# lorenzsp/EMRI_FrequencyDomainWaveforms

Measured on AMD Instinct MI355X. Metric: FD waveforms/sec (2 yr, dt=10 s, ~3000 modes) at 1/2/4/8 GPUs; mode-sum HBM GB/s, higher is better.
Workload: dtype f64

## Files before the change

emri_frequencydomainwaveforms_amd/csrc/emrifd.hip:

```cpp

#include "emrifd_layout.h"

#define EFD_VERSION 100

static thread_local std::string g_err;

int efdhip::fail(int code, const std::string& msg) {
    g_err = msg;
    return code;
}

namespace {

constexpr int NWAVE = TILE / 64;
constexpr int XCD_GROUP = 1024 / TILE;
constexpr int SEGWIN = TILE;
constexpr int PIECES = (int)sizeof(Item) / 16;
constexpr int B_PIECE = (int)offsetof(Item, b) / 16;
constexpr int ROUNDS = 2;
constexpr int NC = (ROUNDS * TILE) / PIECES;


__device__ __forceinline__ bool seg_hits_tile(int2 lh, int32_t tlo, int32_t thi) {
    return lh.y > tlo && lh.x < thi;
}

struct HitRecords {
    int p0, count;
};
__device__ __forceinline__ HitRecords hit_records(
    int sg, int64_t tile, int32_t tlo, int32_t thi, const int32_t* __restrict__ segbase,
    const int32_t* __restrict__ stb0, const int32_t* __restrict__ stb1,
    const int4* __restrict__ seginfo, const int4* __restrict__ ranges) {
    const int32_t sbase = segbase[sg];
    if (sbase != SEG_NO_STB) {
        const int q0 = stb0[sbase + tile], q1 = stb1[sbase + tile];
        return {q0, max(q1 - q0, 0)};
    }
    const int4 info = seginfo[sg];
    const int base = info.x, n = info.y, dir = info.z, sb = info.w;
    int lo = 0, hi = n;
    while (lo < hi) {
        const int mid = (lo + hi) >> 1;
        const int4 rg = ranges[base + (dir > 0 ? mid : n - 1 - mid)];
        if ((sb ? rg.w : rg.y) > tlo) hi = mid; else lo = mid + 1;
    }
    const int p0 = lo;
    hi = n;
    while (lo < hi) {
// ... 232 lines not shown
    const uint64_t m = x >= 64 ? ~0ull : ((1ull << (x & 63)) - 1ull);
    return x <= 0 ? 0ull : m;
}
__device__ __forceinline__ uint64_t lane_range_mask(int32_t lo, int32_t hi) {
    return lanes_below(hi) & ~lanes_below(lo);
}
struct RecSign {
    int32_t fdcls;
    int32_t shift;
    double kth;
    bool safe;
};
__device__ __forceinline__ RecSign rec_sign(uint32_t bits) {
    const bool fdneg = bits & 1u;
    RecSign r;
    r.safe = (bits & 2u) != 0;
    r.fdcls = fdneg ? 0x018 : 0x180;
    r.shift = fdneg ? -192 : 192;
    r.kth = fdneg ? -KTH0 / VS : KTH0 / VS;
    return r;
}
__device__ __forceinline__ uint64_t class_mask(double x, int32_t cls) {
    uint64_t m;
    asm volatile("v_cmp_class_f64_e64 %0, %1, %2" : "=s"(m) : "v"(x), "s"(cls));
    return m;
}
__device__ __forceinline__ double ftz_select(bool ok, double v) {
    return __hiloint2double(ok ? __double2hiint(v) : 0, __double2loint(v));
}
constexpr int HDR_HB = TILE_LANES < 1024 ? 10 : 11;
constexpr uint32_t HDR_HM = (1u << HDR_HB) - 1u;
constexpr int HDR_S = 2 * HDR_HB, HDR_J = 2 * HDR_HB + 1, HDR_FD = 2 * HDR_HB + 4;
static_assert(FAST_J < 8, "header: jser in 3 bits");
static_assert(TILE_LANES < 2048 && HDR_FD + 2 <= 32, "header: one 32-bit word");
__device__ __forceinline__ uint32_t hdr_pack(uint32_t lo, uint32_t hi, int s, int32_t jser,
                                             int32_t fdneg) {
    return lo | (hi << HDR_HB) | ((uint32_t)s << HDR_S) | ((uint32_t)jser << HDR_J) |
           ((uint32_t)fdneg << HDR_FD);
}
__device__ __forceinline__ int32_t hdr_lo(uint32_t ha) { return (int32_t)(ha & HDR_HM); }
__device__ __forceinline__ int32_t hdr_hi(uint32_t ha) {
    return (int32_t)((ha >> HDR_HB) & HDR_HM);
}
__device__ __forceinline__ int hdr_s(uint32_t ha) { return (int)((ha >> HDR_S) & 1u); }
__device__ __forceinline__ uint32_t hdr_jser(uint32_t ha) { return (ha >> HDR_J) & 7u; }
__device__ __forceinline__ uint32_t hdr_fdneg(uint32_t ha) { return (ha >> HDR_FD) & 3u; }
__device__ __forceinline__ uint32_t hdr_safe(uint32_t ha) { return (ha >> (HDR_FD + 1)) & 1u; }
__device__ __forceinline__ bool hdr_test(uint32_t ha, uint32_t mask) {
    asm volatile("" : "+s"(ha));
    return (ha & mask) != 0;
}
__device__ __forceinline__ bool hdr_j3(uint32_t ha) {
    asm volatile("" : "+s"(ha));
    return hdr_jser(ha) >= 3u;
}
__device__ __forceinline__ bool hdr_j4(uint32_t ha) {
    asm volatile("" : "+s"(ha));
    return hdr_jser(ha) >= 4u;
}
__device__ __forceinline__ void spa_simple(const Item* __restrict__ it, double sfk, double stfk,
                                           const double2* __restrict__ sct, const RecSign& rs,
                                           double& wr, double& wi, double& w) {
    const double u = sfk - it->gx;
    const double tt = fma(fma(fma(it->ic[0], u, it->ic[1]), u, it->ic[2]), u, it->ic[3]);
    w = tt - it->tj;
    const double ph = fma(fma(fma(it->ph[0], w, it->ph[1]), w, it->ph[2]), w, it->ph[3]);
    const double fd = fma(fma(it->fd[0], w, it->fd[1]), w, it->fd[2]);
// ... 340 lines not shown
#pragma unroll
            for (int rd = 0; rd < KEYCAP / (4 * TILE); ++rd) {
                const int pc = rd * TILE + tid;
                if (4 * pc < pre)
                    glds16(reinterpret_cast<const uint4*>(tkeys + (size_t)tile * KEYCAP) + pc,
                           reinterpret_cast<uint4*>(keys) + rd * TILE + wave * 64);
            }
        }
#pragma unroll
        for (int rd = 0; rd < SCTAB / TILE; ++rd)
            glds16(reinterpret_cast<const uint4*>(sctab_g) + rd * TILE + tid,
                   reinterpret_cast<uint4*>(sctab) + rd * TILE + wave * 64);
        __builtin_amdgcn_s_waitcnt(0x0f70);
        __syncthreads();
    }

    const int32_t w_lo = (int32_t)(tile * TILE_LANES + wave * 64 * BPL);
    const int32_t e_lo = w_lo + 64 * ioff;
    const int32_t e_hi = e_lo + 64 * NB;
    double fk[NB], tfk[NB];
    double own_r[NB], own_i[NB], mir_r[NB], mir_i[NB];
#pragma unroll
    for (int i = 0; i < NB; ++i) {
        const int32_t k = e_lo + 64 * i + lane;
        fk[i] = (anyrec && k < nlanes) ? freq[k] : 0.0;
        tfk[i] = TWO_PI * fk[i];
        own_r[i] = own_i[i] = mir_r[i] = mir_i[i] = 0.0;
    }
    int s_cur = 0;
#pragma unroll
    for (int i = 0; i < NB; ++i) { fk[i] = -fk[i]; tfk[i] = -tfk[i]; }

    static_assert(PIECES * NC <= ROUNDS * TILE, "staging: at most ROUNDS 16-B pieces per thread");
#define EFD_GLDS(c, buf)                                                                      \
    do {                                                                                      \
        _Pragma("unroll") for (int rd_ = 0; rd_ < ROUNDS; ++rd_) {                            \
            const int p_ = rd_ * TILE + tid;                                                  \
            const int r_ = p_ / PIECES, q_ = p_ - r_ * PIECES;                                \
            if (r_ < NC && (c) * NC + r_ < cnt) {                                             \
                const uint32_t key_ = keys[(c) * NC + r_];                                    \
                 \
                       \
                const int qs_ = ((key_ & 1u) && q_ >= B_PIECE && q_ < B_PIECE + 8)            \
                                    ? ((q_ - B_PIECE + 4) & 7) + B_PIECE : q_;                \
                const uint4* src_ = reinterpret_cast<const uint4*>(items + (key_ >> 1)) + qs_; \
                uint4* dst_ = reinterpret_cast<uint4*>(&stage[(buf)][0]) + rd_ * TILE + wave * 64; \
                glds16(src_, dst_);                                                           \
            }                                                                                 \
        }                                                                                     \
    } while (0)

    int win = 0;
    int nhit = 0;
    int wtotal = 0;
    int wdone = 0;
    int nkeys = pre > 0 ? pre : 0;
    while (true) {
        while (pre < 0 && nkeys < KEYCAP) {
            tid = opq(tid0);
            lane = tid & 63;
            if (wdone == wtotal) {
                if (win >= nseg) break;
                constexpr int ROWS = SEGWIN / TILE;
                unsigned long long bal[ROWS];
#pragma unroll
                for (int row = 0; row < ROWS; ++row) {
                    const int sgi = win + row * TILE + tid;
                    bool hit = false;
                    if (sgi < nseg) hit = seg_hits_tile(seglh[sgi], tlo, thi);
                    bal[row] = __ballot(hit);
                    if (lane == 0) wcnt[row * NWAVE + wave] = __popcll(bal[row]);
                }
                __syncthreads();
                nhit = 0;
#pragma unroll
                for (int row = 0; row < ROWS; ++row) {
                    int before = nhit;
// ... 117 lines not shown
#pragma unroll
                        for (int i = 0; i < NB; ++i) need[i] = false;
                    } else
                    if (CAUSTIC == EFD_CAUSTIC_UNIFORM &&
                        !hdr_test(((uint32_t)((e_lo - klo) | (khi - e_hi)) >> 31) |
                                  ((hdr_jser(ha) + 5u) >> 3) |
                                  (hdr_safe(ha) ^ 1u), 1u)) {
#pragma unroll
                        for (int i = 0; i < NB; ++i) {
                            spa_simple(it, fk[i], tfk[i], sctab, rs, wr[i], wi[i], w[i]);
                            need[i] = false;
                        }
                    } else
                    if (CAUSTIC == EFD_CAUSTIC_UNIFORM &&
                        !hdr_test(((uint32_t)((e_lo - klo) | (khi - e_hi)) >> 31) |
                                  (((hdr_jser(ha) ^ 3u) + 7u) >> 3) |
                                  (hdr_safe(ha) ^ 1u), 1u)) {
#pragma unroll
                        for (int i = 0; i < NB; ++i) {
                            spa_simple3(it, fk[i], tfk[i], sctab, rs, wr[i], wi[i], w[i]);
                            need[i] = false;
                        }
                    } else
#pragma unroll
                    for (int i = 0; i < NB; ++i) {
                        const int32_t base = e_lo + 64 * i;
                        const uint64_t am = lane_range_mask(klo - base, khi - base);
                        spa_fast_m<CAUSTIC>(it, fk[i], tfk[i], ha, am, sctab, rs,
                                            wr[i], wi[i], w[i], needm[i]);
                        need[i] = __builtin_amdgcn_inverse_ballot_w64(needm[i]);
                        needany |= needm[i];
                    }
                    anyneed = needany != 0;
#pragma unroll
                    for (int i = 0; i < NB; ++i) {
                        const double xr = cubic(xo, w[i]), xi = cubic(xo + 4, w[i]);
                        own_r[i] = fma(xr, wr[i], own_r[i]);
                        own_r[i] = fma(-xi, wi[i], own_r[i]);
                        own_i[i] = fma(xr, wi[i], own_i[i]);
                        own_i[i] = fma(xi, wr[i], own_i[i]);
                    }
                    if (PAIRED) {
                        asm volatile("" ::: "memory");
#pragma unroll
                        for (int i = 0; i < NB; ++i) {
                            const double zr = cubic(xm, w[i]), zi = cubic(xm + 4, w[i]);
                            mir_r[i] = fma(zr, wr[i], mir_r[i]);
                            mir_r[i] = fma(-zi, wi[i], mir_r[i]);
                            mir_i[i] = fma(-zr, wi[i], mir_i[i]);
                            mir_i[i] = fma(-zi, wr[i], mir_i[i]);
                        }
                    }
                    if (__builtin_expect(anyneed, 0)) {
                        EFD_EXP_DO(exp_cold(need, lane);)
                        const uint32_t key = rfl(keys[c * NC + ii]);
                        const int hg = (int)((key >> 1) / (uint32_t)ni);
                        const int jr = (int)((key >> 1) - (uint32_t)hg * (uint32_t)ni);
                        const int ln = opq(tid0) & 63;
#pragma unroll
                        for (int i = 0; i < NB; ++i) {
                            if (need[i]) {
                                const double f = freq[e_lo + 64 * i + ln];
                                const ColdEval ce = spa_general<CAUSTIC>(
                                    it, s_cur ? f : -f, s, hg, jr, t, nt, K, gm, gn, coefA, coefT);
                                accumulate<0, PAIRED>(ce.wr, ce.wi, ce.b[0], ce.b[1], ce.b[2],
                                                      ce.b[3], own_r[i], own_i[i], mir_r[i],
                                                      mir_i[i]);
                            }
                        }
                        {
                            const int ln2 = opq(tid0) & 63;
#pragma unroll
                            for (int i = 0; i < NB; ++i) {
                                const int32_t k = e_lo + 64 * i + ln2;
                                const double f = k < nlanes ? freq[k] : 0.0;
// ... 1343 lines not shown
```

emri_frequencydomainwaveforms_amd/csrc/emrifd_cpu.cpp:

```cpp
#include <algorithm>
#include <cmath>
#include <cstdint>
#include <cstdio>
#include <cstdlib>
#include <cstring>
#include <numeric>
#include <string>
#include <vector>

#include <omp.h>

#include "../../include/emrifd.h"
#include "emrifd_cpu_internal.h"

namespace efdcpu {

struct double2 {
    double x, y;
};
#define EFD_TABLE static const
#include "spa_tables.inc"
#undef EFD_TABLE

#include "emrifd_constants.h"
// ... 248 lines not shown
                spline_nak(npts, [&](int q) { return knotF(a->f_phi, a->f_r, m, n, KI(q)); },
                           [&](int q) { return a->t[KI(q)]; },
                           reinterpret_cast<double(*)[4]>(ti.data()), c1, d1, s1);
                for (int q = 0; q < npts - 1; ++q) {
                    const int jf = sg > 0 ? ra + q : rb - 1 - q;
                    for (int c = 0; c < 4; ++c) R[jf].ic[c] = ti[(size_t)q * 4 + c];
                    R[jf].gx = knotF(a->f_phi, a->f_r, m, n, KI(q));
                }
                const double dm = (double)m, dn = (double)n;
                for (int j = ra; j < rb; ++j) {
                    Rec& it = R[j];
                    it.tj = a->t[j];
                    it.dtj = a->t[j + 1] - a->t[j];
                    for (int c = 0; c < 4; ++c) {
                        const double* ca = P.coefA.data() + ((size_t)j * 4 + c) * 4 * G + 4 * g;
                        it.b[0][0][c] = ca[0]; it.b[0][1][c] = ca[1];
                        it.b[1][0][c] = ca[2]; it.b[1][1][c] = ca[3];
                        const double* ct = P.coefT.data() + ((size_t)j * 4 + c) * 8;
                        it.ph[c] = dm * ct[0] + dn * ct[1];
                    }
                    const double* ct = P.coefT.data() + (size_t)j * 32;
                    const double F0 = dm * ct[2] + dn * ct[3], F1 = dm * ct[10] + dn * ct[11],
                                 F2 = dm * ct[18] + dn * ct[19];
                    it.fd[0] = 3.0 * F0; it.fd[1] = 2.0 * F1; it.fd[2] = F2;
                    const double G0 = dm * ct[4] + dn * ct[5], G1 = dm * ct[12] + dn * ct[13],
                                 G2 = dm * ct[20] + dn * ct[21];
                    it.fdd[0] = FDD_SCALE * (3.0 * G0);
                    it.fdd[1] = FDD_SCALE * (2.0 * G1);
                    it.fdd[2] = FDD_SCALE * G2;
                    const double dt = it.dtj;
                    auto qv = [](double p0, double p1, double p2, double x) { return (p0 * x + p1) * x + p2; };
                    const double fa = it.fd[2], fb = qv(it.fd[0], it.fd[1], it.fd[2], dt);
                    it.fdneg = qv(it.fd[0], it.fd[1], it.fd[2], 0.5 * dt) < 0.0 ? 1 : 0;
                    double fdmin = std::fmin(std::fabs(fa), std::fabs(fb));
                    if ((fa > 0.0) != (fb > 0.0) || fa == 0.0 || fb == 0.0) fdmin = 0.0;
                    if (it.fd[0] != 0.0) {
                        const double xv = -it.fd[1] / (2.0 * it.fd[0]);
                        if (xv > 0.0 && xv < dt) {
                            const double fv = qv(it.fd[0], it.fd[1], it.fd[2], xv);
                            if ((fv > 0.0) != (fa > 0.0)) fdmin = 0.0;
                            fdmin = std::fmin(fdmin, std::fabs(fv));
                        }
                    }
                    double gmax = std::fmax(std::fabs(G2), std::fabs(qv(3.0 * G0, 2.0 * G1, G2, dt)));
                    if (G0 != 0.0) {
                        const double xv = -(2.0 * G1) / (6.0 * G0);
                        if (xv > 0.0 && xv < dt) gmax = std::fmax(gmax, std::fabs(qv(3.0 * G0, 2.0 * G1, G2, xv)));
                    }
                    const double ymin = gmax > 0.0 ? TWO_PI * fdmin * fdmin * fdmin / (3.0 * gmax * gmax) / 1.1
                                                   : INFINITY;
                    int J = FAST_J;
                    for (int jj = 1; jj < FAST_J; ++jj)
                        if (ymin >= JSER_Y[jj]) { J = jj; break; }
                    it.jser = J;
                    it.envc = 0;
                    if (env_on && ymin >= ENV_MIN_Y) {
                        const double gq[3] = {3.0 * G0, 2.0 * G1, G2};
                        EnvFit E;
                        if (env_fit(it.fd, gq, it.dtj, (it.fdneg & 1) != 0, E)) {
                            it.envc = 1;
                            for (int c = 0; c <= ENV_DEG; ++c) it.env[c] = E.a[c];
                            for (int c = 0; c < 4; ++c) it.phE[c] = it.ph[c] - E.th[c];
                        }
                    }
                    const double Fj = knotF(a->f_phi, a->f_r, m, n, j);
                    const double Fj1 = knotF(a->f_phi, a->f_r, m, n, j + 1);
// ... 135 lines not shown
                       dm * ct[20] + dn * ct[21]);
    }
    xo[0] = b[2 * s]; xo[1] = b[2 * s + 1];
    zo[0] = b[2 - 2 * s]; zo[1] = b[3 - 2 * s];
    const double amp = fd != 0.0 ? 1.0 / std::sqrt(std::fabs(fd)) : 0.0;
    const double psi = std::fma(TWO_PI * g, tt, -ph) + (fd > 0.0 ? 0.75 * PI : -0.75 * PI);
    double R = 1.0, I = 0.0;
    if (caustic == EFD_CAUSTIC_UNIFORM && fd != 0.0 && fdd != 0.0) {
        const double a2 = amp * amp;
        const double ww = (fd > 0.0 ? 1.0 : -1.0) * (3.0 / TWO_PI) * fdd * fdd * a2 * a2 * a2;
        if (std::fabs(ww) * FAST_Y <= 1.0) {
            const double uu = ww * ww;
            double r = KB[FAST_J - 1], im = KC[FAST_J - 1];
            for (int j = FAST_J - 2; j >= 0; --j) {
                r = std::fma(r, uu, KB[j]);
                im = std::fma(im, uu, KC[j]);
            }
            R = r;
            I = ww * im;
        } else {
            kfactor_slow(fd, fdd, R, I);
        }
    }
    const double sn = std::sin(psi), cs = std::cos(psi);
    wr = amp * (R * cs - I * sn);
    wi = amp * (R * sn + I * cs);
}

template <int CAUSTIC, bool J34>
void spa_fast(const Rec& it, int s, const double* fk, int n, double* wr, double* wi, double* wv,
              unsigned char* need) {
    const SinCosTable& T = sctab();
    const double sgn = s ? 1.0 : -1.0;
    const bool neg = it.fdneg != 0;
    const int shift = neg ? -192 : 192;
    const double kth = neg ? -KTH0 / VS : KTH0 / VS;
    constexpr double INV_STEP = 81.48733086305042;
    constexpr double STEP_1 = 0.01227184630308513;
    constexpr double SHIFTER = 6755399441055744.0;
#pragma omp simd
    for (int i = 0; i < n; ++i) {
        const double g = sgn * fk[i];
        const double u = g - it.gx;
        const double tt = std::fma(std::fma(std::fma(it.ic[0], u, it.ic[1]), u, it.ic[2]), u, it.ic[3]);
        const double w = tt - it.tj;
        bool good = (w >= 0.0) & (w < it.dtj);
        const double ph = std::fma(std::fma(std::fma(it.ph[0], w, it.ph[1]), w, it.ph[2]), w, it.ph[3]);
        const double fd = std::fma(std::fma(it.fd[0], w, it.fd[1]), w, it.fd[2]);
        good = good & (neg ? (fd < 0.0) & (fd > -INFINITY) : (fd > 0.0) & (fd < INFINITY));
        const double ampm = good ? 1.0 / std::sqrt(std::fabs(fd)) : 0.0;
        const double psi0 = std::fma(TWO_PI * g, tt, -ph);
        double am = ampm, c0 = COS_A, thn = 0.0, ksc = 0.0;
        if (CAUSTIC == EFD_CAUSTIC_UNIFORM) {
            const double fdds = std::fma(std::fma(it.fdd[0], w, it.fdd[1]), w, it.fdd[2]);
            const double a3 = ampm * ampm * ampm;
            const double t3 = fdds * a3;
            double ww = t3 * t3;
            if (J34) {
                const bool inr = ww <= VS / FAST_Y;
                good = good & inr;
                ww = inr ? ww : 0.0;
                const double uu = ww * ww;
                const double r = std::fma(45.7, uu * uu, 1.0 - uu);
                thn = ww * std::fma(-14.733333333333333333, uu, 1.0);
                am = good ? ampm * r : 0.0;
            } else {
                c0 = std::fma(-ww, ww, COS_A);
// ... 269 lines not shown
```

emri_frequencydomainwaveforms_amd/csrc/emrifd_layout.h:

```cpp
#pragma once

#include "emrifd_common.h"

namespace {

#include "emrifd_constants.h"

constexpr int TILE_LANES = TILE * BPL;
constexpr int SEG1_NT = 1024;
constexpr int SEG1_MAX_K = SEG1_NT / (2 * MAXRUNS);
constexpr int KEYCAP = 2048;
constexpr int SPLIT_ITEM_CAP = 8192;
constexpr int SPLIT_TILE_CAP = 128;
constexpr int SPLIT_UNION_CAP = 4096;
constexpr int SPLIT_MIN_COST = 48;
constexpr int SPLIT_SLOTS_PER_WF = 64;

#define EFD_TABLE __constant__
#include "spa_tables.inc"
__device__ __forceinline__ double env_rsqrt(double x) {
    double y = __builtin_amdgcn_rsq(x);
    y = y * fma(-0.5 * x * y, y, 1.5);
    return y * fma(-0.5 * x * y, y, 1.5);
}
#define EFD_HD __device__
#include "env_fit.inc"
#undef EFD_HD


struct __attribute__((aligned(16))) Item {
    double gx;
    double ic[4];
    double tj;
    double ph[4];
    double fd[3];
    double dtj;
    double fdd[3];
    int32_t jser;
    int32_t fdneg;
    double b[2][2][4];
    int32_t klo[2], khi[2];
};
static_assert(sizeof(Item) == 288, "Item must be 288 B");
static_assert(offsetof(Item, dtj) == offsetof(Item, fd) + 24 &&
              offsetof(Item, fdd) == offsetof(Item, fd) + 32 &&
              offsetof(Item, jser) == offsetof(Item, fd) + 8 * (ENV_DEG + 1),
              "envelope coefficients: fd, dtj, fdd contiguous");
constexpr double ENV_AMP_SCALE = 1.000000000029531;
__host__ __device__ __forceinline__ double* env_of(Item* it) {
    return reinterpret_cast<double*>(reinterpret_cast<char*>(it) + offsetof(Item, fd));
}
__host__ __device__ __forceinline__ const double* env_of(const Item* it) {
    return reinterpret_cast<const double*>(reinterpret_cast<const char*>(it) + offsetof(Item, fd));
}
static_assert(offsetof(Item, ph) % 16 == 0 && offsetof(Item, fd) % 16 == 0 &&
              offsetof(Item, fdd) % 16 == 0, "the fast path's coefficient pairs are 16-B aligned");
static_assert(offsetof(Item, b) % 16 == 0 && sizeof(Item::b) == 8 * 16, "b: 8 whole pieces");

constexpr int64_t HDR_MAGIC = 0x45464448445233LL;
struct Header {
    int64_t contributions;
    int64_t evaluations;
    int32_t runs_overflow;
    int32_t groups;
    int32_t bad_mn;
    int32_t bad_tile;
    int64_t magic;
    int32_t lane_lo, lane_hi;
    int32_t nitems;
    int32_t nsplit;
    int64_t env_evaluations;
};
static_assert(sizeof(Header) == 64, "Header must be 64 B");


struct Layout {
// ... 125 lines not shown
```

emri_frequencydomainwaveforms_amd/csrc/emrifd_prepare.hip:

```cpp

#include "emrifd_layout.h"

namespace {

constexpr int SPLINE_PF = 8;

__device__ __forceinline__ double spl_rcp(double x) {
#ifdef EFD_EXP_EXACT_RCP
    return 1.0 / x;
#endif
    double y = __builtin_amdgcn_rcp(x);
    double e = fma(-x, y, 1.0);
    y = fma(y, e, y);
    e = fma(-x, y, 1.0);
    return fma(y, e, y);
}

template <class FX, class FY, class FCP, class FDP, class FOUT>
__device__ void spline_not_a_knot(int n, FX X, FY Y, FCP CP, FDP DP, FOUT OUT) {
    if (n < 2) return;
    if (n == 2) {
        const double dx = X(1) - X(0);
        const double slope = (Y(1) - Y(0)) / dx;
        OUT(0, 0, 0.0); OUT(0, 1, 0.0); OUT(0, 2, slope); OUT(0, 3, Y(0));
// ... 967 lines not shown
    };
    const double wa = wat(ga), wb = wat(gb);
    const double mg = 1e-6 * it.dtj;
    if (!(fmin(wa, wb) >= mg && fmax(wa, wb) <= it.dtj - mg)) return false;
    const double ua = ga - it.gx, ub = gb - it.gx;
    auto dt = [&](double u) { return fma(fma(3.0 * it.ic[0], u, 2.0 * it.ic[1]), u, it.ic[2]); };
    const double da = dt(ua), db = dt(ub);
    if (!((da > 0.0 && db > 0.0) || (da < 0.0 && db < 0.0))) return false;
    if (it.ic[0] != 0.0) {
        const double uv = -it.ic[1] / (3.0 * it.ic[0]);
        if (uv > ua && uv < ub) {
            const double dv = dt(uv);
            if (!((dv > 0.0) == (da > 0.0) && dv != 0.0)) return false;
        }
    }
    const double* f = it.fd;
    const double scale = fabs(f[0]) * it.dtj * it.dtj + fabs(f[1]) * it.dtj + fabs(f[2]);
    const double sg = (it.fdneg & 1) ? -1.0 : 1.0;
    auto fq = [&](double x) { return sg * fma(fma(f[0], x, f[1]), x, f[2]); };
    double fmn = fmin(fq(0.0), fq(it.dtj));
    if (f[0] != 0.0) {
        const double xv = -f[1] / (2.0 * f[0]);
        if (xv > 0.0 && xv < it.dtj) fmn = fmin(fmn, fq(xv));
    }
    return fmn > 1e-12 * scale && isfinite(scale);
}

__device__ bool build_item(
    const double* __restrict__ t, const double* __restrict__ f_phi, const double* __restrict__ f_r,
    const int32_t* __restrict__ gm, const int32_t* __restrict__ gn, int ni, int K,
    const double* __restrict__ coefA, const double* __restrict__ coefT,
    const int32_t* __restrict__ runs, const double* __restrict__ freq, int64_t nf, int paired,
    int64_t nl, int64_t nl1, Item* __restrict__ items, int4* __restrict__ ranges, int h, int j,
    unsigned long long& evals, bool env) {
    Item& it = items[(size_t)h * ni + j];
    const int m = gm[h], n = gn[h];
    const int32_t* rr = runs + (size_t)h * 4 * MAXRUNS;
    int run = -1;
    for (int r = 0; r < MAXRUNS; ++r) {
        if (rr[4 * r + 2] != 0 && j >= rr[4 * r] && j < rr[4 * r + 1]) { run = r; break; }
    }
    const int partner = (m != 0) ? 1 : 0;
    evals = 0;
    it.fdneg = 0;
    if (run < 0) {
        it.klo[0] = it.khi[0] = it.klo[1] = it.khi[1] = 0;
        ranges[(size_t)h * ni + j] = make_int4(0, 0, 0, 0);
        return false;
    }
    const int a = rr[4 * run], sg = rr[4 * run + 2];
    it.tj = t[j];
    it.dtj = t[j + 1] - t[j];
    const double dm = (double)m, dn = (double)n;
    for (int c = 0; c < 4; ++c) {
        const double* ca = coefA + ((size_t)j * 4 + c) * 4 * K + 4 * h;
        it.b[0][0][c] = ca[0];
        it.b[0][1][c] = ca[1];
        it.b[1][0][c] = ca[2];
        it.b[1][1][c] = ca[3];
        const double* ct = coefT + ((size_t)j * 4 + c) * 8;
        it.ph[c] = dm * ct[0] + dn * ct[1];
    }
    double gq[3], ymin_rec;
    {
        const double* ct = coefT + (size_t)j * 32;
        const double F0 = dm * ct[0 * 8 + 2] + dn * ct[0 * 8 + 3];
        const double F1 = dm * ct[1 * 8 + 2] + dn * ct[1 * 8 + 3];
        const double F2 = dm * ct[2 * 8 + 2] + dn * ct[2 * 8 + 3];
        it.fd[0] = 3.0 * F0; it.fd[1] = 2.0 * F1; it.fd[2] = F2;
        const double G0 = dm * ct[0 * 8 + 4] + dn * ct[0 * 8 + 5];
        const double G1 = dm * ct[1 * 8 + 4] + dn * ct[1 * 8 + 5];
        const double G2 = dm * ct[2 * 8 + 4] + dn * ct[2 * 8 + 5];
        it.fdd[0] = FDD_SCALE * (3.0 * G0);
        it.fdd[1] = FDD_SCALE * (2.0 * G1);
        it.fdd[2] = FDD_SCALE * G2;
        const double dt = it.dtj;
        auto qv = [](double a, double b, double c, double x) { return (a * x + b) * x + c; };
        const double fa = it.fd[2], fb = qv(it.fd[0], it.fd[1], it.fd[2], dt);
        it.fdneg = qv(it.fd[0], it.fd[1], it.fd[2], 0.5 * dt) < 0.0 ? 1 : 0;
        double fdmin = fmin(fabs(fa), fabs(fb));
        if ((fa > 0.0) != (fb > 0.0) || fa == 0.0 || fb == 0.0) fdmin = 0.0;
        if (it.fd[0] != 0.0) {
            const double xv = -it.fd[1] / (2.0 * it.fd[0]);
            if (xv > 0.0 && xv < dt) {
                const double fv = qv(it.fd[0], it.fd[1], it.fd[2], xv);
                if ((fv > 0.0) != (fa > 0.0)) fdmin = 0.0;
                fdmin = fmin(fdmin, fabs(fv));
            }
        }
        double gmax = fmax(fabs(G2), fabs(qv(3.0 * G0, 2.0 * G1, G2, dt)));
        if (G0 != 0.0) {
            const double xv = -(2.0 * G1) / (6.0 * G0);
            if (xv > 0.0 && xv < dt) gmax = fmax(gmax, fabs(qv(3.0 * G0, 2.0 * G1, G2, xv)));
        }
        const double ymin = gmax > 0.0 ? TWO_PI * fdmin * fdmin * fdmin / (3.0 * gmax * gmax) / 1.1
                                       : INFINITY;
        int J = FAST_J;
        for (int jj = 1; jj < FAST_J; ++jj)
            if (ymin >= JSER_Y[jj]) { J = jj; break; }
        it.jser = J;
        gq[0] = 3.0 * G0; gq[1] = 2.0 * G1; gq[2] = G2;
        ymin_rec = ymin;
    }
    const double Fj = knotF_rn(f_phi, f_r, m, n, j), Fj1 = knotF_rn(f_phi, f_r, m, n, j + 1);
    const double xlo = sg > 0 ? Fj : Fj1;
    const double xhi = sg > 0 ? Fj1 : Fj;
    const bool strict_lo = sg > 0 ? (j == a) : (j + 1 == rr[4 * run + 1]);
    const double f0 = freq[0], span = freq[nf - 1] - f0;
    const double gsc = span > 0.0 ? (double)(nf - 1) / span : 0.0;
    auto guess = [&](double v) { return (int64_t)floor((v - f0) * gsc); };
    const double bv[4] = {-xhi, -xlo, xlo, xhi};
    const bool bu[4] = {true, !strict_lo, strict_lo, false};
// ... 21 lines not shown
        if (!(g >= 1 && pred(b3[q][0]))) {
            if (g == nf) k = nf;
            else if (pred(b3[q][1])) k = g;
            else if (g + 1 == nf) k = nf;
            else if (pred(b3[q][2])) k = g + 1;
        }
        if (k < 0)
            k = bu[q] ? grid_bound<true>(freq, nf, v, g) : grid_bound<false>(freq, nf, v, g);
        bk[q] = k;
    }
    int64_t lo0 = bk[0], hi0 = bk[1], lo1 = bk[2], hi1 = bk[3];
    const int64_t lim0 = paired ? nl : nf;
    const int64_t lim1 = paired ? nl1 : (partner ? nf : 0);
    auto clampr = [](int64_t& lo, int64_t& hi, int64_t lim) {
        if (lo > lim) lo = lim;
        if (hi > lim) hi = lim;
        if (hi < lo) hi = lo;
    };
    clampr(lo0, hi0, lim0);
    clampr(lo1, hi1, lim1);
    it.klo[0] = (int32_t)lo0; it.khi[0] = (int32_t)hi0;
    it.klo[1] = (int32_t)lo1; it.khi[1] = (int32_t)hi1;
    ranges[(size_t)h * ni + j] = make_int4((int)lo0, (int)hi0, (int)lo1, (int)hi1);
    auto fat = [&](int q, int64_t x) {
        const int64_t g = bg[q];
        if (g >= 1 && x == g - 1) return b3[q][0];
        if (g < nf && x == g) return b3[q][1];
        if (g + 1 < nf && x == g + 1) return b3[q][2];
        return freq[x];
    };
    if (record_safe(it, fat, lo0, hi0, lo1, hi1)) it.fdneg |= 2;
    const int mult = paired ? 1 + partner : 1;
    evals = (unsigned long long)((hi0 - lo0) + (hi1 - lo1)) * mult;
    if (env && (it.fdneg & 2) && ymin_rec >= ENV_MIN_Y && evals > 0) {
        EnvFit E;
        if (env_fit(it.fd, gq, it.dtj, (it.fdneg & 1) != 0, E)) {
            double* e = env_of(&it);
            for (int c = 0; c <= ENV_DEG; ++c) e[c] = E.a[c] * ENV_AMP_SCALE;
            for (int c = 0; c < 4; ++c) it.ph[c] -= E.th[c];
            it.jser = 0;
            return true;
        }
    }
    return false;
}

__device__ __forceinline__ void items_body(const double* __restrict__ t, const double* __restrict__ f_phi,
                        const double* __restrict__ f_r, const int32_t* __restrict__ gm,
                        const int32_t* __restrict__ gn, const int32_t* __restrict__ gstart,
                        int nt, int K, const double* __restrict__ coefA,
                        const double* __restrict__ coefT, const int32_t* __restrict__ runs,
                        const double* __restrict__ freq, int64_t nf, int paired, int64_t nl,
                        int64_t nl1, Item* __restrict__ items, int4* __restrict__ ranges,
                        Header* __restrict__ hdr, bool runs_mark, bool env) {
    const int ni = nt - 1;
    const int G = hdr->groups;
    const int64_t total = (int64_t)ni * G;
    if ((int64_t)blockIdx.x * blockDim.x >= total) return;
    const int64_t stride = (int64_t)gridDim.x * blockDim.x;
    __shared__ unsigned long long red[3][4];
    unsigned long long ev = 0, contrib = 0, eev = 0;
    for (int64_t gid = (int64_t)blockIdx.x * blockDim.x + threadIdx.x; gid < total;
         gid += stride) {
        const int g = (int)(gid % G), j = (int)(gid / G);
        if (runs_mark && j == 0 && runs[(size_t)g * 4 * MAXRUNS + 3] != 0)
            atomicOr(&hdr->runs_overflow, 1);
        unsigned long long e1 = 0;
        const bool envr = build_item(t, f_phi, f_r, gm, gn, ni, K, coefA, coefT, runs, freq, nf,
                                     paired, nl, nl1, items, ranges, g, j, e1, env);
        ev += e1;
        contrib += e1 * (unsigned long long)(gstart[g + 1] - gstart[g]);
        eev += envr ? e1 : 0;
    }
    for (int o = 32; o > 0; o >>= 1) {
        ev += __shfl_xor(ev, o);
        contrib += __shfl_xor(contrib, o);
        eev += __shfl_xor(eev, o);
    }
    if ((threadIdx.x & 63) == 0) {
        red[0][threadIdx.x >> 6] = contrib;
        red[1][threadIdx.x >> 6] = ev;
        red[2][threadIdx.x >> 6] = eev;
    }
    __syncthreads();
    if (threadIdx.x == 0) {
        const unsigned long long c = red[0][0] + red[0][1] + red[0][2] + red[0][3];
        const unsigned long long e = red[1][0] + red[1][1] + red[1][2] + red[1][3];
        const unsigned long long x = red[2][0] + red[2][1] + red[2][2] + red[2][3];
        if (c) atomicAdd((unsigned long long*)&hdr->contributions, c);
        if (e) atomicAdd((unsigned long long*)&hdr->evaluations, e);
        if (x) atomicAdd((unsigned long long*)&hdr->env_evaluations, x);
    }
}
__global__ __launch_bounds__(256) void k_items(const PrepBatch B) {
    const PrepView V(B);
    items_body(V.t, V.f_phi, V.f_r, V.gm, V.gn, V.gstart, V.nt, V.K, V.coefA, V.coefT, V.runs,
               V.freq, V.nf, V.paired, V.nl, V.nl1, V.items, V.ranges, V.header,
               (V.pcr & 1) != 0, V.env != 0);
}

__device__ __forceinline__ void slot_segment(const PrepView& V, int i,
                                             const int4* __restrict__ ranges, int G, int2& lh,
                                             int4& info) {
    const int h = i / (2 * MAXRUNS), r = (i >> 1) % MAXRUNS, sb = i & 1;
    const int ni = V.nt - 1;
    lh = make_int2(0, 0);
    info = make_int4(0, 0, 0, 0);
    const int32_t* rr = V.runs + (size_t)h * 4 * MAXRUNS + 4 * r;
    if (h < G && rr[2] != 0) {
        const int ja = rr[0], jb = rr[1], n = jb - ja;
        const int dir = (sb == 0) ? -rr[2] : rr[2];
        const int lim = V.seg_lim(sb);
        const int4* rg = ranges + (size_t)h * ni;
        int lo = 0, hi = n;
        while (lo < hi) {
            const int mid = (lo + hi) >> 1;
            const int4 v = rg[dir > 0 ? ja + mid : jb - 1 - mid];
            if ((sb ? v.w : v.y) > 0) hi = mid; else lo = mid + 1;
        }
        const int pa = lo;
        hi = n;
        while (lo < hi) {
            const int mid = (lo + hi) >> 1;
            const int4 v = rg[dir > 0 ? ja + mid : jb - 1 - mid];
            if ((sb ? v.z : v.x) >= lim) hi = mid; else lo = mid + 1;
        }
        const int pb = lo;
        if (pb > pa) {
            const int4 rf = rg[dir > 0 ? ja + pa : jb - 1 - pa];
            const int4 rl = rg[dir > 0 ? ja + pb - 1 : jb - pb];
            const int klo = sb ? rf.z : rf.x, khi = sb ? rl.w : rl.y;
            if (khi > klo) {
                lh = make_int2(klo, khi);
                const int jfirst = dir > 0 ? ja + pa : jb - pb;
                info = make_int4(h * ni + jfirst, pb - pa, dir, sb);
            }
        }
    }
}
__device__ __forceinline__ int slot_blocks(int K) { return (2 * MAXRUNS * K + 255) / 256; }
__global__ __launch_bounds__(256) void k_segment_slots(const PrepBatch B) {
    const PrepView V(B);
    if ((int)blockIdx.x >= slot_blocks(V.K)) return;
    const int i = blockIdx.x * blockDim.x + threadIdx.x;
    __shared__ int wc[4], wt[4];
    int ntl = 0;
    bool valid = false;
    if (i < V.K * MAXRUNS * 2) {
        int2 lh;
        int4 info;
        slot_segment(V, i, V.ranges, V.header->groups, lh, info);
        V.slotlh[i] = lh;
        V.slotinfo[i] = info;
        valid = info.y > 0;
        if (valid) ntl = (lh.y - 1) / TILE_LANES - lh.x / TILE_LANES + 1;
    }
    const unsigned long long bal = __ballot(valid);
    int tsum = ntl;
    for (int o = 32; o > 0; o >>= 1) tsum += __shfl_xor(tsum, o);
    if ((threadIdx.x & 63) == 0) {
        wc[threadIdx.x >> 6] = __popcll(bal);
        wt[threadIdx.x >> 6] = tsum;
    }
    __syncthreads();
    if (threadIdx.x == 0) {
        V.slotcnt[blockIdx.x] = wc[0] + wc[1] + wc[2] + wc[3];
        V.slottiles[blockIdx.x] = wt[0] + wt[1] + wt[2] + wt[3];
    }
}

__global__ __launch_bounds__(256) void k_segment_compact(const PrepBatch B) {
    const PrepView V(B);
    const int nblk = slot_blocks(V.K), nslot = 2 * MAXRUNS * V.K;
    if ((int)blockIdx.x >= nblk) return;
    Header* hdr = V.header;
    __shared__ int wc[4];
    __shared__ int64_t wt[4];
    __shared__ int2 wr[4];
    const int tid = threadIdx.x, lane = tid & 63, wave = tid >> 6;
    const int blk = blockIdx.x;
    int before = 0;
    int64_t tbefore = 0;
    for (int b = tid; b < blk; b += 256) { before += V.slotcnt[b]; tbefore += V.slottiles[b]; }
    for (int o = 32; o > 0; o >>= 1) {
        before += __shfl_xor(before, o);
        tbefore += __shfl_xor(tbefore, o);
    }
    if (lane == 0) { wc[wave] = before; wt[wave] = tbefore; }
    __syncthreads();
    const int base = wc[0] + wc[1] + wc[2] + wc[3];
    const int64_t tbase = wt[0] + wt[1] + wt[2] + wt[3];
    __syncthreads();
    const int i = blk * 256 + tid;
    int4 info = make_int4(0, 0, 0, 0);
    int2 lh = make_int2(0, 0);
    if (i < nslot) { info = V.slotinfo[i]; lh = V.slotlh[i]; }
    const bool valid = info.y > 0;
    const int ntl = valid ? (lh.y - 1) / TILE_LANES - lh.x / TILE_LANES + 1 : 0;
    int incl = ntl;
    for (int o = 1; o < 64; o <<= 1) {
        const int v = __shfl_up(incl, o, 64);
        if (lane >= o) incl += v;
    }
    const unsigned long long bal = __ballot(valid);
    if (lane == 63) wt[wave] = incl;
    if (lane == 0) wc[wave] = __popcll(bal);
    __syncthreads();
    int pos = base;
    int64_t toff = tbase + incl - ntl;
    for (int w = 0; w < wave; ++w) { pos += wc[w]; toff += wt[w]; }
    pos += __popcll(bal & ((1ull << lane) - 1ull));
    if (valid) {
        V.seglh[pos] = lh;
        V.seginfo[pos] = info;
        V.segbase[pos] = (toff + ntl <= V.stbcap) ? (int32_t)(toff - lh.x / TILE_LANES)
                                                  : SEG_NO_STB;
    }
    if (blk == nblk - 1 && tid == 0) *V.nseg = base + wc[0] + wc[1] + wc[2] + wc[3];
    int lo = valid ? lh.x : INT32_MAX, hi = valid ? lh.y : INT32_MIN;
    for (int o = 32; o > 0; o >>= 1) {
        lo = min(lo, __shfl_xor(lo, o));
        hi = max(hi, __shfl_xor(hi, o));
    }
    if (lane == 0) wr[wave] = make_int2(lo, hi);
    __syncthreads();
    if (tid == 0) {
        for (int w = 1; w < 4; ++w) { lo = min(lo, wr[w].x); hi = max(hi, wr[w].y); }
        if (lo < hi) {
            atomicMin(&hdr->lane_lo, lo);
            atomicMax(&hdr->lane_hi, hi);
        }
    }
}

__device__ __forceinline__ int div_floor_nn(int64_t a) { return (int)(a / TILE_LANES); }
__device__ __forceinline__ void seg_tiles_record(const int4* __restrict__ ranges, int2 lh,
                                                 int4 info, int32_t sbase, int p,
                                                 int32_t* __restrict__ stb0,
                                                 int32_t* __restrict__ stb1) {
    const int base = info.x, n = info.y, dir = info.z, sb = info.w;
    const int t0 = lh.x / TILE_LANES, t1 = (lh.y - 1) / TILE_LANES;
    auto rng = [&](int q) {
        const int4 rg = ranges[base + (dir > 0 ? q : n - 1 - q)];
        return sb ? make_int2(rg.z, rg.w) : make_int2(rg.x, rg.y);
    };
    const int2 cur = p < n ? rng(p) : make_int2(0, 0);
    const int2 prv = p > 0 ? rng(p - 1) : make_int2(0, 0);
    int a = p > 0 ? (int)((prv.y + TILE_LANES - 1) / TILE_LANES) : t0;
    int b = p < n ? (cur.y > 0 ? div_floor_nn(cur.y - 1) : -1) : t1;
    for (int t = max(a, t0); t <= min(b, t1); ++t) stb0[sbase + t] = p;
    a = p > 0 ? div_floor_nn(prv.x) : t0;
// ... 142 lines not shown
    if (n_split == 0 || n_items > SPLIT_ITEM_CAP || n_split > SPLIT_TILE_CAP)
        return;
    int4* items = V.sitem;
    int32_t* cnt = V.scnt;
    int ii = io, sp = po;
    for (int i = 0; i < PER; ++i) {
        const int u = tid * PER + i, S = nS[i];
        for (int j = 0; j < S; ++j)
            items[ii + j] = make_int4(ut0 + u, (j << 16) | S, S > 1 ? sp : -1, S > 1 ? sp : -1);
        if (S > 1) {
            cnt[sp] = 0;
            ++sp;
        }
        ii += S;
    }
    if (tid == 0) {
        hdr->nitems = n_items;
        hdr->nsplit = n_split;
    }
}

}

static int32_t split_min_cost() {
    const char* e = getenv("EFD_SPLIT_MIN_COST");
    if (!e || !*e) return SPLIT_MIN_COST;
    const long long x = atoll(e);
    return x >= -1 && x <= (1 << 30) ? (int32_t)x : SPLIT_MIN_COST;
}

static bool env_records() {
    static const bool v = [] {
        const char* e = std::getenv("EFD_ENV");
        return !(e && e[0] == '0');
    }();
    return v;
}

static int fill_desc(const std::string& F, const efd_modesum_args* const* a,
                     void* const* workspace, const size_t* workspace_bytes, int i, PrepDesc& d,
                     Layout& L) {
    const efd_modesum_args* ai = a[i];
    const int rc = efdhip::check_modesum_args(ai, workspace[i], 1);
    if (rc != EFD_OK) return rc;
    if (ai->nf != a[0]->nf || (ai->grid_symmetric != 0) != (a[0]->grid_symmetric != 0))
        return fail(EFD_ERR_ARG, F + ": nf and grid_symmetric must agree across the batch");
    L = make_layout(ai->nt, ai->K, ai->nf, ai->grid_symmetric ? 1 : 0);
    if (workspace_bytes[i] < L.total)
        return fail(EFD_ERR_WORKSPACE, F + ": workspace too small (see "
                                           "efd_modesum_workspace_bytes)");
    for (int j = 0; j < i; ++j)
        if (workspace[j] == workspace[i])
            return fail(EFD_ERR_ARG, F + ": one workspace per waveform");
    d.t = ai->t; d.phi_phi = ai->phi_phi; d.phi_r = ai->phi_r; d.f_phi = ai->f_phi;
    d.f_r = ai->f_r; d.amp = ai->amp; d.ylm_p = ai->ylm_p; d.ylm_m = ai->ylm_m;
    d.freq = ai->freq; d.m = ai->m; d.n = ai->n;
    d.ws = (char*)workspace[i];
    d.sc_re = ai->scale_re; d.sc_im = ai->scale_im;
    d.nt = ai->nt; d.K = ai->K;
    d.lists = efdhip::list_mode(ai->K, L.ntiles);
    d.env = (ai->caustic == EFD_CAUSTIC_UNIFORM && env_records()) ? 1 : 0;
#ifdef EFD_EXP_NO_PCR
    const bool pcr = false;
#else
    const bool pcr = ai->nt >= 4 && ai->nt <= PCR_NMAX;
#endif
    d.pcr = pcr ? (ai->K < PCR_MAX_K ? 3 : 1) : 0;
    return EFD_OK;
}

struct PrepShape {
    int ntmax = 0, Kmax = 0, ntmax_pcr = 0, pcr_blocks = 0;
    int64_t items_max = 0, seg_lds = 0;
    bool any_pcr = false, any_thomas = false, any_lists = false, any_order = false;
    void add(const PrepDesc& d) {
        any_lists |= d.lists != 0;
        any_order |= d.lists == 3;
        if (d.pcr) {
            any_pcr = true;
            ntmax_pcr = std::max(ntmax_pcr, d.nt);
            pcr_blocks = std::max(pcr_blocks, 4 + (d.pcr == 3 ? 5 : 1) * d.K);
        }
        if (d.pcr != 3) any_thomas = true;
        ntmax = std::max(ntmax, d.nt);
        Kmax = std::max(Kmax, d.K);
        const int64_t per = d.K >= ITEMS_SPLIT_K ? ITEMS_PER_THREAD_K : 1;
        items_max = std::max(items_max, ((int64_t)(d.nt - 1) * d.K + per - 1) / per);
        const int64_t b = (int64_t)d.K * (d.nt - 1) * 16;
        if (b <= SEG1_LDS_CAP) seg_lds = std::max(seg_lds, b);
    }
};

static int launch_chain(PrepBatch& B, const PrepShape& S, int64_t ntiles, hipStream_t st) {
    const unsigned nz = (unsigned)B.n;
// ... 130 lines not shown
```

Measured before the change: 1843.

## Skip partnerless own/mirror accumulation, reorder segment slots, precompute staging indices

Items whose mode has no paired partner are tagged with a new fdneg bit at prepare time. The mode-sum kernel then skips the own or mirror accumulation loop, depending on the sign bit, for those items, instead of adding zero-weight contributions. The segment slots are also reordered so the two slot halves are dense, and the second half is padded to a SEGWIN boundary so windows do not straddle halves. The per-thread staging indices for the global-to-LDS copy are precomputed into a packed register, replacing per-round divisions and selects. This adds header-bit coupling and extra padding segments, and it is gated by the EFD_PARTNER_SKIP environment variable, which defaults on.

```diff
diff --git a/emri_frequencydomainwaveforms_amd/csrc/emrifd.hip b/emri_frequencydomainwaveforms_amd/csrc/emrifd.hip
--- a/emri_frequencydomainwaveforms_amd/csrc/emrifd.hip
+++ b/emri_frequencydomainwaveforms_amd/csrc/emrifd.hip
@@ -14,7 +14,6 @@
 
 constexpr int NWAVE = TILE / 64;
 constexpr int XCD_GROUP = 1024 / TILE;
-constexpr int SEGWIN = TILE;
 constexpr int PIECES = (int)sizeof(Item) / 16;
 constexpr int B_PIECE = (int)offsetof(Item, b) / 16;
 constexpr int ROUNDS = 2;
@@ -313,7 +312,9 @@
 constexpr uint32_t HDR_HM = (1u << HDR_HB) - 1u;
 constexpr int HDR_S = 2 * HDR_HB, HDR_J = 2 * HDR_HB + 1, HDR_FD = 2 * HDR_HB + 4;
 static_assert(FAST_J < 8, "header: jser in 3 bits");
-static_assert(TILE_LANES < 2048 && HDR_FD + 2 <= 32, "header: one 32-bit word");
+constexpr int HDR_NP = HDR_FD + 2;
+static_assert(TILE_LANES < 2048 && HDR_FD + 3 <= 32, "header: one 32-bit word");
+static_assert(ITEM_NO_PARTNER == 1 << (HDR_NP - HDR_FD), "header: Item::fdneg's bits in place");
 __device__ __forceinline__ uint32_t hdr_pack(uint32_t lo, uint32_t hi, int s, int32_t jser,
                                              int32_t fdneg) {
     return lo | (hi << HDR_HB) | ((uint32_t)s << HDR_S) | ((uint32_t)jser << HDR_J) |
@@ -720,17 +721,27 @@
     for (int i = 0; i < NB; ++i) { fk[i] = -fk[i]; tfk[i] = -tfk[i]; }
 
     static_assert(PIECES * NC <= ROUNDS * TILE, "staging: at most ROUNDS 16-B pieces per thread");
+    static_assert(NC < 32 && PIECES <= 32 && 12 * ROUNDS <= 32, "staging: 12 bits per round");
+    uint32_t glpack = 0;
+#pragma unroll
+    for (int rd = 0; rd < ROUNDS; ++rd) {
+        const int p = rd * TILE + tid0;
+        const int r = p / PIECES, q = p - r * PIECES;
+        const int d = (q >= B_PIECE && q < B_PIECE + 8) ? (q < B_PIECE + 4 ? 1 : -1) : 0;
+        glpack |= ((uint32_t)min(r, NC) | ((uint32_t)q << 5) | ((uint32_t)(d & 3) << 10))
+                  << (12 * rd);
+    }
 #define EFD_GLDS(c, buf)                                                                      \
     do {                                                                                      \
+        const uint32_t g_ = (uint32_t)opq((int)glpack);                                       \
+        const int rem_ = min(NC, cnt - (c) * NC);                                             \
         _Pragma("unroll") for (int rd_ = 0; rd_ < ROUNDS; ++rd_) {                            \
-            const int p_ = rd_ * TILE + tid;                                                  \
-            const int r_ = p_ / PIECES, q_ = p_ - r_ * PIECES;                                \
-            if (r_ < NC && (c) * NC + r_ < cnt) {                                             \
+            const int r_ = (int)((g_ >> (12 * rd_)) & 31u);                                   \
+            if (r_ < rem_) {                                                                  \
                 const uint32_t key_ = keys[(c) * NC + r_];                                    \
-                 \
-                       \
-                const int qs_ = ((key_ & 1u) && q_ >= B_PIECE && q_ < B_PIECE + 8)            \
-                                    ? ((q_ - B_PIECE + 4) & 7) + B_PIECE : q_;                \
+                const int q_ = (int)((g_ >> (12 * rd_ + 5)) & 31u);                           \
+                const int d_ = (int)(g_ << (20 - 12 * rd_)) >> 30;                            \
+                const int qs_ = q_ + 4 * d_ * (int)(key_ & 1u);                               \
                 const uint4* src_ = reinterpret_cast<const uint4*>(items + (key_ >> 1)) + qs_; \
                 uint4* dst_ = reinterpret_cast<uint4*>(&stage[(buf)][0]) + rd_ * TILE + wave * 64; \
                 glds16(src_, dst_);                                                           \
@@ -914,6 +925,7 @@
                         needany |= needm[i];
                     }
                     anyneed = needany != 0;
+                    if (!hdr_test((ha >> HDR_NP) & (ha >> HDR_S), 1u))
 #pragma unroll
                     for (int i = 0; i < NB; ++i) {
                         const double xr = cubic(xo, w[i]), xi = cubic(xo + 4, w[i]);
@@ -922,7 +934,7 @@
                         own_i[i] = fma(xr, wi[i], own_i[i]);
                         own_i[i] = fma(xi, wr[i], own_i[i]);
                     }
-                    if (PAIRED) {
+                    if (PAIRED && !hdr_test((ha >> HDR_NP) & ~(ha >> HDR_S), 1u)) {
                         asm volatile("" ::: "memory");
 #pragma unroll
                         for (int i = 0; i < NB; ++i) {
diff --git a/emri_frequencydomainwaveforms_amd/csrc/emrifd_cpu.cpp b/emri_frequencydomainwaveforms_amd/csrc/emrifd_cpu.cpp
--- a/emri_frequencydomainwaveforms_amd/csrc/emrifd_cpu.cpp
+++ b/emri_frequencydomainwaveforms_amd/csrc/emrifd_cpu.cpp
@@ -304,6 +304,7 @@
                     auto qv = [](double p0, double p1, double p2, double x) { return (p0 * x + p1) * x + p2; };
                     const double fa = it.fd[2], fb = qv(it.fd[0], it.fd[1], it.fd[2], dt);
                     it.fdneg = qv(it.fd[0], it.fd[1], it.fd[2], 0.5 * dt) < 0.0 ? 1 : 0;
+                    if (!partner) it.fdneg |= 4;
                     double fdmin = std::fmin(std::fabs(fa), std::fabs(fb));
                     if ((fa > 0.0) != (fb > 0.0) || fa == 0.0 || fb == 0.0) fdmin = 0.0;
                     if (it.fd[0] != 0.0) {
@@ -505,7 +506,7 @@
               unsigned char* need) {
     const SinCosTable& T = sctab();
     const double sgn = s ? 1.0 : -1.0;
-    const bool neg = it.fdneg != 0;
+    const bool neg = (it.fdneg & 1) != 0;
     const int shift = neg ? -192 : 192;
     const double kth = neg ? -KTH0 / VS : KTH0 / VS;
     constexpr double INV_STEP = 81.48733086305042;
diff --git a/emri_frequencydomainwaveforms_amd/csrc/emrifd_layout.h b/emri_frequencydomainwaveforms_amd/csrc/emrifd_layout.h
--- a/emri_frequencydomainwaveforms_amd/csrc/emrifd_layout.h
+++ b/emri_frequencydomainwaveforms_amd/csrc/emrifd_layout.h
@@ -10,6 +10,7 @@
 constexpr int SEG1_NT = 1024;
 constexpr int SEG1_MAX_K = SEG1_NT / (2 * MAXRUNS);
 constexpr int KEYCAP = 2048;
+constexpr int SEGWIN = TILE;
 constexpr int SPLIT_ITEM_CAP = 8192;
 constexpr int SPLIT_TILE_CAP = 128;
 constexpr int SPLIT_UNION_CAP = 4096;
@@ -42,6 +43,7 @@
     int32_t klo[2], khi[2];
 };
 static_assert(sizeof(Item) == 288, "Item must be 288 B");
+constexpr int32_t ITEM_NO_PARTNER = 4;
 static_assert(offsetof(Item, dtj) == offsetof(Item, fd) + 24 &&
               offsetof(Item, fdd) == offsetof(Item, fd) + 32 &&
               offsetof(Item, jser) == offsetof(Item, fd) + 8 * (ENV_DEG + 1),
diff --git a/emri_frequencydomainwaveforms_amd/csrc/emrifd_prepare.hip b/emri_frequencydomainwaveforms_amd/csrc/emrifd_prepare.hip
--- a/emri_frequencydomainwaveforms_amd/csrc/emrifd_prepare.hip
+++ b/emri_frequencydomainwaveforms_amd/csrc/emrifd_prepare.hip
@@ -1023,7 +1023,7 @@
     const double* __restrict__ coefA, const double* __restrict__ coefT,
     const int32_t* __restrict__ runs, const double* __restrict__ freq, int64_t nf, int paired,
     int64_t nl, int64_t nl1, Item* __restrict__ items, int4* __restrict__ ranges, int h, int j,
-    unsigned long long& evals, bool env) {
+    unsigned long long& evals, int env) {
     Item& it = items[(size_t)h * ni + j];
     const int m = gm[h], n = gn[h];
     const int32_t* rr = runs + (size_t)h * 4 * MAXRUNS;
@@ -1069,6 +1069,7 @@
         auto qv = [](double a, double b, double c, double x) { return (a * x + b) * x + c; };
         const double fa = it.fd[2], fb = qv(it.fd[0], it.fd[1], it.fd[2], dt);
         it.fdneg = qv(it.fd[0], it.fd[1], it.fd[2], 0.5 * dt) < 0.0 ? 1 : 0;
+        if (!partner && (env & 2)) it.fdneg |= ITEM_NO_PARTNER;
         double fdmin = fmin(fabs(fa), fabs(fb));
         if ((fa > 0.0) != (fb > 0.0) || fa == 0.0 || fb == 0.0) fdmin = 0.0;
         if (it.fd[0] != 0.0) {
@@ -1156,7 +1157,7 @@
     if (record_safe(it, fat, lo0, hi0, lo1, hi1)) it.fdneg |= 2;
     const int mult = paired ? 1 + partner : 1;
     evals = (unsigned long long)((hi0 - lo0) + (hi1 - lo1)) * mult;
-    if (env && (it.fdneg & 2) && ymin_rec >= ENV_MIN_Y && evals > 0) {
+    if ((env & 1) && (it.fdneg & 2) && ymin_rec >= ENV_MIN_Y && evals > 0) {
         EnvFit E;
         if (env_fit(it.fd, gq, it.dtj, (it.fdneg & 1) != 0, E)) {
             double* e = env_of(&it);
@@ -1176,7 +1177,7 @@
                         const double* __restrict__ coefT, const int32_t* __restrict__ runs,
                         const double* __restrict__ freq, int64_t nf, int paired, int64_t nl,
                         int64_t nl1, Item* __restrict__ items, int4* __restrict__ ranges,
-                        Header* __restrict__ hdr, bool runs_mark, bool env) {
+                        Header* __restrict__ hdr, bool runs_mark, int env) {
     const int ni = nt - 1;
     const int G = hdr->groups;
     const int64_t total = (int64_t)ni * G;
@@ -1220,7 +1221,7 @@
     const PrepView V(B);
     items_body(V.t, V.f_phi, V.f_r, V.gm, V.gn, V.gstart, V.nt, V.K, V.coefA, V.coefT, V.runs,
                V.freq, V.nf, V.paired, V.nl, V.nl1, V.items, V.ranges, V.header,
-               (V.pcr & 1) != 0, V.env != 0);
+               (V.pcr & 1) != 0, V.env);
 }
 
 __device__ __forceinline__ void slot_segment(const PrepView& V, int i,
@@ -1263,6 +1264,10 @@
     }
 }
 __device__ __forceinline__ int slot_blocks(int K) { return (2 * MAXRUNS * K + 255) / 256; }
+__device__ __forceinline__ int dense_slot(int i, int K) {
+    const int half = MAXRUNS * K, sb = i >= half ? 1 : 0;
+    return 2 * (i - sb * half) + sb;
+}
 __global__ __launch_bounds__(256) void k_segment_slots(const PrepBatch B) {
     const PrepView V(B);
     if ((int)blockIdx.x >= slot_blocks(V.K)) return;
@@ -1273,7 +1278,7 @@
     if (i < V.K * MAXRUNS * 2) {
         int2 lh;
         int4 info;
-        slot_segment(V, i, V.ranges, V.header->groups, lh, info);
+        slot_segment(V, dense_slot(i, V.K), V.ranges, V.header->groups, lh, info);
         V.slotlh[i] = lh;
         V.slotinfo[i] = info;
         valid = info.y > 0;
@@ -1297,24 +1302,38 @@
     const PrepView V(B);
     const int nblk = slot_blocks(V.K), nslot = 2 * MAXRUNS * V.K;
     if ((int)blockIdx.x >= nblk) return;
+    static_assert(SEGWIN <= 256, "one workgroup writes the padding");
     Header* hdr = V.header;
-    __shared__ int wc[4];
+    __shared__ int wc[4], wn[4], wa[4];
     __shared__ int64_t wt[4];
     __shared__ int2 wr[4];
     const int tid = threadIdx.x, lane = tid & 63, wave = tid >> 6;
     const int blk = blockIdx.x;
-    int before = 0;
+    const int half = nslot / 2, bs = half / 256;
+    int before = 0, n0 = 0, all = 0;
     int64_t tbefore = 0;
-    for (int b = tid; b < blk; b += 256) { before += V.slotcnt[b]; tbefore += V.slottiles[b]; }
+    for (int b = tid; b < nblk; b += 256) {
+        const int c = V.slotcnt[b];
+        all += c;
+        if (b < bs) n0 += c;
+        if (b < blk) { before += c; tbefore += V.slottiles[b]; }
+    }
+    if (bs * 256 + tid < half && V.slotinfo[bs * 256 + tid].y > 0) ++n0;
     for (int o = 32; o > 0; o >>= 1) {
         before += __shfl_xor(before, o);
+        n0 += __shfl_xor(n0, o);
+        all += __shfl_xor(all, o);
         tbefore += __shfl_xor(tbefore, o);
     }
-    if (lane == 0) { wc[wave] = before; wt[wave] = tbefore; }
+    if (lane == 0) { wc[wave] = before; wn[wave] = n0; wa[wave] = all; wt[wave] = tbefore; }
     __syncthreads();
     const int base = wc[0] + wc[1] + wc[2] + wc[3];
+    const int nseg0 = wn[0] + wn[1] + wn[2] + wn[3];
+    const int nsegs = wa[0] + wa[1] + wa[2] + wa[3];
     const int64_t tbase = wt[0] + wt[1] + wt[2] + wt[3];
     __syncthreads();
+    int pad = (SEGWIN - nseg0 % SEGWIN) % SEGWIN;
+    if (nseg0 == nsegs || nsegs + pad > nslot) pad = 0;
     const int i = blk * 256 + tid;
     int4 info = make_int4(0, 0, 0, 0);
     int2 lh = make_int2(0, 0);
@@ -1330,7 +1349,7 @@
     if (lane == 63) wt[wave] = incl;
     if (lane == 0) wc[wave] = __popcll(bal);
     __syncthreads();
-    int pos = base;
+    int pos = base + (i >= half ? pad : 0);
     int64_t toff = tbase + incl - ntl;
     for (int w = 0; w < wave; ++w) { pos += wc[w]; toff += wt[w]; }
     pos += __popcll(bal & ((1ull << lane) - 1ull));
@@ -1340,7 +1359,12 @@
         V.segbase[pos] = (toff + ntl <= V.stbcap) ? (int32_t)(toff - lh.x / TILE_LANES)
                                                   : SEG_NO_STB;
     }
-    if (blk == nblk - 1 && tid == 0) *V.nseg = base + wc[0] + wc[1] + wc[2] + wc[3];
+    if (blk == bs && tid < pad) {
+        V.seglh[nseg0 + tid] = make_int2(0, 0);
+        V.seginfo[nseg0 + tid] = make_int4(0, 0, 0, 0);
+        V.segbase[nseg0 + tid] = SEG_NO_STB;
+    }
+    if (blk == nblk - 1 && tid == 0) *V.nseg = nsegs + pad;
     int lo = valid ? lh.x : INT32_MAX, hi = valid ? lh.y : INT32_MIN;
     for (int o = 32; o > 0; o >>= 1) {
         lo = min(lo, __shfl_xor(lo, o));
@@ -1549,6 +1573,14 @@
 static bool env_records() {
     static const bool v = [] {
         const char* e = std::getenv("EFD_ENV");
+        return !(e && e[0] == '0');
+    }();
+    return v;
+}
+
+static bool partner_skip() {
+    static const bool v = [] {
+        const char* e = std::getenv("EFD_PARTNER_SKIP");
         return !(e && e[0] == '0');
     }();
     return v;
@@ -1576,7 +1608,8 @@
     d.sc_re = ai->scale_re; d.sc_im = ai->scale_im;
     d.nt = ai->nt; d.K = ai->K;
     d.lists = efdhip::list_mode(ai->K, L.ntiles);
-    d.env = (ai->caustic == EFD_CAUSTIC_UNIFORM && env_records()) ? 1 : 0;
+    d.env = ((ai->caustic == EFD_CAUSTIC_UNIFORM && env_records()) ? 1 : 0) |
+            (partner_skip() ? 2 : 0);
 #ifdef EFD_EXP_NO_PCR
     const bool pcr = false;
 #else
```

Result: no change. 1866 (median of 6 runs) (+1.3%).
